# tmuird/VAEUNET

Hardware: AMD Instinct MI355X
Metric: images/sec (whole node) at 3x512x512 bs=8/GPU; Dice parity vs CPU ref (higher is better)
Workload: dtype bf16; 1 GPU; UNet(3,2) train step (fwd+CombinedLoss+bwd+clip+AdamW), random-init weights; image=3x512x512, batch_per_gpu=8, global_batch=8, parallelism=dp1, execution=hipgraph-replay, wgrad_side_stream=False

## Files before the change

vaeunet_amd/csrc/bn.hip:

```cpp
#include <cstdlib>
#include <type_traits>

#include "host.h"

namespace {

constexpr int STATS_TPB = 32;
constexpr int STATS_MAXS = 256;

__global__ void bn_stats_stage1(const float* psum, const float* pm2, int tiles, int64_t tile_rows,
                                int64_t rows, int C, int S, double* ws) {
  __shared__ double sh[4][64];
  const int cl = threadIdx.x & 63, tl = threadIdx.x >> 6;
  const int c = blockIdx.x * 64 + cl;
  const bool ok = c < C;
  const int per = (tiles + S - 1) / S;
  const int tb0 = blockIdx.y * per, te0 = min(tiles, tb0 + per);
  constexpr int U = STATS_TPB / 4;
  double N = 0, Mn = 0, Q = 0;
  for (int tb = tb0; tb < te0; tb += STATS_TPB) {
    const int te = min(te0, tb + STATS_TPB);
    const int64_t n_r = min(rows, (int64_t)te * tile_rows) - (int64_t)tb * tile_rows;
    float sv[U], mv[U];
    double nv[U];
    const int cc = ok ? c : 0;
#pragma unroll
    for (int u = 0; u < U; ++u) {
      const int t = min(tb + tl + 4 * u, te - 1);
      sv[u] = psum[(int64_t)t * C + cc];
      mv[u] = pm2[(int64_t)t * C + cc];
    }
#pragma unroll
    for (int u = 0; u < U; ++u) {
      const int t = tb + tl + 4 * u;
      const bool in = ok && t < te;
      sv[u] = in ? sv[u] : 0.f;
      mv[u] = in ? mv[u] : 0.f;
      int64_t nt = rows - (int64_t)t * tile_rows;
      nv[u] = in ? (double)(nt > tile_rows ? tile_rows : nt) : 0.0;
    }
    double s = 0;
#pragma unroll
    for (int u = 0; u < U; ++u) s += (double)sv[u];
    sh[tl][cl] = s;
    __syncthreads();
    const double m = (sh[0][cl] + sh[1][cl] + sh[2][cl] + sh[3][cl]) / (double)n_r;
    __syncthreads();
    double q = 0;
#pragma unroll
    for (int u = 0; u < U; ++u) {
      if (nv[u] > 0) {
        const double d = (double)sv[u] / nv[u] - m;
        q += (double)mv[u] + nv[u] * d * d;
      }
    }
    sh[tl][cl] = q;
// ... 41 lines not shown
  }
  double n = 0, sm = 0;
#pragma unroll
  for (int u = 0; u < U; ++u) { n += nv[u]; sm += nv[u] * mv[u]; }
  sh[0][q][cl] = n; sh[1][q][cl] = sm;
  __syncthreads();
#pragma unroll
  for (int w = 16; w >= 1; w >>= 1) {
    if (q < w) { sh[0][q][cl] += sh[0][q + w][cl]; sh[1][q][cl] += sh[1][q + w][cl]; }
    __syncthreads();
  }
  n = sh[0][0][cl];
  const double m = n > 0 ? sh[1][0][cl] / n : 0.0;
  __syncthreads();
  double M2 = 0;
#pragma unroll
  for (int u = 0; u < U; ++u) { const double d = mv[u] - m; M2 += qv[u] + nv[u] * d * d; }
  sh[0][q][cl] = M2;
  __syncthreads();
#pragma unroll
  for (int w = 16; w >= 1; w >>= 1) {
    if (q < w) sh[0][q][cl] += sh[0][q + w][cl];
    __syncthreads();
  }
  if (q != 0 || !ok) return;
  M2 = sh[0][0][cl];
  double var = n > 0 ? M2 / n : 0.0;
  float invstd = (float)(1.0 / sqrt(var + (double)eps));
  float mean = (float)m;
  scale[c] = g * invstd;
  shift[c] = b - mean * g * invstd;
  if (smean) smean[c] = mean;
  if (sinvstd) sinvstd[c] = invstd;
  if (nbt && c == 0) nbt[0] = nb0 + 1;
  if (upd) {
    double unb = n > 1 ? M2 / (n - 1) : var;
    rmean[c] = (1.f - momentum) * rm0 + momentum * mean;
    rvar[c] = (1.f - momentum) * rv0 + momentum * (float)unb;
  }
}

__global__ void bn_eval_kernel(const float* gamma, const float* beta, const float* rm, const float* rv,
                               float eps, int C, float* scale, float* shift, float* smean, float* sinvstd) {
  int c = blockIdx.x * blockDim.x + threadIdx.x;
  if (c >= C) return;
  float invstd = 1.f / sqrtf(rv[c] + eps);
  float g = gamma ? gamma[c] : 1.f, b = beta ? beta[c] : 0.f;
  scale[c] = g * invstd;
  shift[c] = b - rm[c] * g * invstd;
  if (smean) smean[c] = rm[c];
  if (sinvstd) sinvstd[c] = invstd;
}

struct ChanMap {
  int V, R, cv, row;
  VU_DEV ChanMap(int C) {
    V = C >> 3;
    R = 256 / V;
    cv = threadIdx.x & (V - 1);
    row = threadIdx.x / V;
  }
};

constexpr int UNR = 4;

template <typename T, bool NT>
__global__ void bn_apply_kernel(const T* x, int64_t xs, T* y, int64_t ys, int64_t P, int C,
                                const float* scale, const float* shift, int relu) {
  ChanMap cm(C);
  const int c = cm.cv * 8;
  float sc[8], sh[8];
#pragma unroll
  for (int i = 0; i < 8; ++i) { sc[i] = scale[c + i]; sh[i] = shift[c + i]; }
  const int64_t step = (int64_t)gridDim.x * cm.R * UNR;
  for (int64_t p0 = (int64_t)blockIdx.x * cm.R * UNR + cm.row; p0 < P; p0 += step) {
    Vec8<T> v[UNR];
#pragma unroll
    for (int u = 0; u < UNR; ++u) {
      const int64_t p = p0 + (int64_t)u * cm.R;
      if (p < P) { if (NT) v[u].load_nt(x + p * xs + c); else v[u].load(x + p * xs + c); }
    }
#pragma unroll
    for (int u = 0; u < UNR; ++u) {
      const int64_t p = p0 + (int64_t)u * cm.R;
      if (p >= P) continue;
#pragma unroll
      for (int i = 0; i < 8; ++i) {
        float z = v[u].get(i) * sc[i] + sh[i];
        v[u].set(i, relu ? fmaxf(z, 0.f) : z);
      }
      v[u].store(y + p * ys + c);
    }
  }
}

constexpr int RED_MAXBLK = 1024;

struct RedArgs {
  const void* a; int64_t as;
  const void* b; int64_t bs;
  int64_t P; int C;
  const float* scale; const float* shift; const float* mean; const float* invstd;
  int relu;
  float* part;
  int H, W, y0, x0, Hr, Wr;
};

VU_DEV int64_t win_pix(const RedArgs& r, int64_t p) {
  if (r.Hr == 0) return p;
  int64_t j = p % r.Wr, t = p / r.Wr;
  int64_t i = t % r.Hr, n = t / r.Hr;
  return (n * r.H + r.y0 + i) * r.W + r.x0 + j;
}

template <typename T, int MODE, bool NT>
__global__ void chan_partial_kernel(RedArgs r) {
  __shared__ float sh[2][256 * 8];
  ChanMap cm(r.C);
  const int c = cm.cv * 8;
  float s0[8], s1[8], sc[8], sf[8], mu[8], is[8];
#pragma unroll
  for (int i = 0; i < 8; ++i) {
    s0[i] = 0.f; s1[i] = 0.f;
    if (MODE == 1) {
      sc[i] = r.scale[c + i]; sf[i] = r.shift[c + i]; mu[i] = r.mean[c + i]; is[i] = r.invstd[c + i];
    }
  }
  const int64_t step = (int64_t)gridDim.x * cm.R * UNR;
  for (int64_t p0 = (int64_t)blockIdx.x * cm.R * UNR + cm.row; p0 < r.P; p0 += step) {
    Vec8<T> va[UNR], vb[UNR];
#pragma unroll
    for (int u = 0; u < UNR; ++u) {
      const int64_t p = p0 + (int64_t)u * cm.R;
      if (p < r.P) {
        const T* pa = reinterpret_cast<const T*>(r.a) + (MODE == 0 ? win_pix(r, p) : p) * r.as + c;
        const T* pb = reinterpret_cast<const T*>(r.b) + p * r.bs + c;
        if (NT) {
          va[u].load_nt(pa);
          if (MODE == 1) vb[u].load_nt(pb);
        } else {
          va[u].load(pa);
          if (MODE == 1) vb[u].load(pb);
        }
      }
    }
#pragma unroll
    for (int u = 0; u < UNR; ++u) {
      if (p0 + (int64_t)u * cm.R >= r.P) continue;
      if (MODE == 0) {
#pragma unroll
        for (int i = 0; i < 8; ++i) s0[i] += va[u].get(i);
      } else {
#pragma unroll
        for (int i = 0; i < 8; ++i) {
          float xv = vb[u].get(i);
          float dz = va[u].get(i);
          if (r.relu && !(fmaf(xv, sc[i], sf[i]) > 0.f)) dz = 0.f;
          s0[i] += dz;
          s1[i] += dz * ((xv - mu[i]) * is[i]);
        }
      }
    }
  }
#pragma unroll
  for (int i = 0; i < 8; ++i) { sh[0][cm.row * r.C + c + i] = s0[i]; sh[1][cm.row * r.C + c + i] = s1[i]; }
  __syncthreads();
  for (int cc = threadIdx.x; cc < r.C; cc += 256) {
    float a0 = 0.f, a1 = 0.f;
    a0 = lds_sum(&sh[0][cc], cm.R, r.C);
// ... 179 lines not shown
    st1<T>(dx + p * dxs + c, fmaf(coef[c], dz, coef[C + c] * (xv - mean[c])) + coef[2 * C + c]);
  }
}

template <typename T>
__global__ void bn_apply_scalar(const T* x, int64_t xs, T* y, int64_t ys, int64_t P, int C,
                                const float* scale, const float* shift, int relu) {
  int64_t tot = P * C;
  for (int64_t e = (int64_t)blockIdx.x * blockDim.x + threadIdx.x; e < tot;
       e += (int64_t)gridDim.x * blockDim.x) {
    int64_t p = e / C;
    int c = (int)(e - p * C);
    float z = ld1<T>(x + p * xs + c) * scale[c] + shift[c];
    st1<T>(y + p * ys + c, relu ? fmaxf(z, 0.f) : z);
  }
}

template <typename T>
__global__ void bn_apply_maxpool_kernel(const T* y, int64_t ys, T* a, int64_t as, T* pool, int64_t ps, int N,
                                        int H, int W, int C, const float* scale, const float* shift, int relu) {
  ChanMap cm(C);
  const int c = cm.cv * 8;
  float sc[8], sh[8];
#pragma unroll
  for (int i = 0; i < 8; ++i) { sc[i] = scale[c + i]; sh[i] = shift[c + i]; }
  const int Ho = H >> 1, Wo = W >> 1;
  const int64_t Q = (int64_t)N * Ho * Wo;
  for (int64_t q = (int64_t)blockIdx.x * cm.R + cm.row; q < Q; q += (int64_t)gridDim.x * cm.R) {
    const int j = (int)(q % Wo);
    const int64_t t = q / Wo;
    const int i = (int)(t % Ho), n = (int)(t / Ho);
    const int64_t p00 = ((int64_t)n * H + 2 * i) * W + 2 * j;
    Vec8<T> v[4];
#pragma unroll
    for (int k = 0; k < 4; ++k) v[k].load(y + (p00 + (k >> 1) * W + (k & 1)) * ys + c);
    float best[8];
#pragma unroll
    for (int e = 0; e < 8; ++e) best[e] = -INFINITY;
#pragma unroll
    for (int k = 0; k < 4; ++k) {
#pragma unroll
      for (int e = 0; e < 8; ++e) {
        const float z = v[k].get(e) * sc[e] + sh[e];
        v[k].set(e, relu ? fmaxf(z, 0.f) : z);
        const float f = v[k].get(e);
        if (f > best[e] || isnan(f)) best[e] = f;
      }
      v[k].store(a + (p00 + (k >> 1) * W + (k & 1)) * as + c);
    }
    Vec8<T> o;
#pragma unroll
    for (int e = 0; e < 8; ++e) o.set(e, best[e]);
    o.store(pool + q * ps + c);
  }
}

struct PoolBnArgs {
  const void* y; int64_t ys;
  const void* dp; int64_t dps;
  const void* add; int64_t adds;
  int N, H, W, C;
  const float* scale; const float* shift; const float* mean; const float* invstd;
  int relu;
  float* part;
  const float* coef;
  void* dx; int64_t dxs;
};

template <typename T, bool NT>
VU_DEV void pool_window(const PoolBnArgs& r, int64_t q, int c, const float (&sc)[8], const float (&sf)[8],
                        float (&yv)[4][8], float (&dz)[4][8], int64_t& p00) {
  const int Wo = r.W >> 1, Ho = r.H >> 1;
  const int j = (int)(q % Wo);
  const int64_t t = q / Wo;
  const int i = (int)(t % Ho), n = (int)(t / Ho);
  p00 = ((int64_t)n * r.H + 2 * i) * r.W + 2 * j;
  const T* y = reinterpret_cast<const T*>(r.y);
  const T* ad = reinterpret_cast<const T*>(r.add);
  Vec8<T> vy[4], va[4], vg;
#pragma unroll
  for (int k = 0; k < 4; ++k) {
    const int64_t pix = p00 + (k >> 1) * r.W + (k & 1);
    if (NT) vy[k].load_nt(y + pix * r.ys + c); else vy[k].load(y + pix * r.ys + c);
    if (ad) { if (NT) va[k].load_nt(ad + pix * r.adds + c); else va[k].load(ad + pix * r.adds + c); }
  }
  vg.load(reinterpret_cast<const T*>(r.dp) + q * r.dps + c);
  float best[8];
  int arg[8];
#pragma unroll
  for (int e = 0; e < 8; ++e) { best[e] = -INFINITY; arg[e] = 0; }
#pragma unroll
  for (int k = 0; k < 4; ++k)
#pragma unroll
    for (int e = 0; e < 8; ++e) {
      yv[k][e] = vy[k].get(e);
      const float z = fmaf(yv[k][e], sc[e], sf[e]);
      const float f = rnd<T>(r.relu ? fmaxf(z, 0.f) : z);
      if (f > best[e] || isnan(f)) { best[e] = f; arg[e] = k; }
    }
#pragma unroll
  for (int k = 0; k < 4; ++k)
#pragma unroll
    for (int e = 0; e < 8; ++e) {
      float o = ad ? va[k].get(e) : 0.f;
      if (arg[e] == k) o += vg.get(e);
      float d = rnd<T>(o);
      if (r.relu && !(fmaf(yv[k][e], sc[e], sf[e]) > 0.f)) d = 0.f;
      dz[k][e] = d;
    }
}

template <typename T, bool NT>
__global__ void pool_bn_partial_kernel(PoolBnArgs r) {
  __shared__ float sh[2][256 * 8];
  ChanMap cm(r.C);
  const int c = cm.cv * 8;
  float s0[8], s1[8], sc[8], sf[8], mu[8], is[8];
#pragma unroll
  for (int e = 0; e < 8; ++e) {
    s0[e] = 0.f; s1[e] = 0.f;
    sc[e] = r.scale[c + e]; sf[e] = r.shift[c + e]; mu[e] = r.mean[c + e]; is[e] = r.invstd[c + e];
  }
  const int64_t Q = (int64_t)r.N * (r.H >> 1) * (r.W >> 1);
  for (int64_t q = (int64_t)blockIdx.x * cm.R + cm.row; q < Q; q += (int64_t)gridDim.x * cm.R) {
    float yv[4][8], dz[4][8];
    int64_t p00;
    pool_window<T, NT>(r, q, c, sc, sf, yv, dz, p00);
#pragma unroll
    for (int k = 0; k < 4; ++k)
#pragma unroll
      for (int e = 0; e < 8; ++e) {
        s0[e] += dz[k][e];
        s1[e] += dz[k][e] * ((yv[k][e] - mu[e]) * is[e]);
      }
  }
#pragma unroll
  for (int e = 0; e < 8; ++e) { sh[0][cm.row * r.C + c + e] = s0[e]; sh[1][cm.row * r.C + c + e] = s1[e]; }
  __syncthreads();
  for (int cc = threadIdx.x; cc < r.C; cc += 256) {
    float a0 = 0.f, a1 = 0.f;
    a0 = lds_sum(&sh[0][cc], cm.R, r.C);
    a1 = lds_sum(&sh[1][cc], cm.R, r.C);
    r.part[((int64_t)blockIdx.x * 2 + 0) * r.C + cc] = a0;
    r.part[((int64_t)blockIdx.x * 2 + 1) * r.C + cc] = a1;
  }
}

template <typename T, bool NT>
__global__ void pool_bn_apply_kernel(PoolBnArgs r) {
  ChanMap cm(r.C);
  const int c = cm.cv * 8;
  float sc[8], sf[8], mu[8], k1[8], k2[8], k3[8];
#pragma unroll
  for (int e = 0; e < 8; ++e) {
    sc[e] = r.scale[c + e]; sf[e] = r.shift[c + e]; mu[e] = r.mean[c + e];
    k1[e] = r.coef[c + e]; k2[e] = r.coef[r.C + c + e]; k3[e] = r.coef[2 * r.C + c + e];
  }
  T* dx = reinterpret_cast<T*>(r.dx);
  const int64_t Q = (int64_t)r.N * (r.H >> 1) * (r.W >> 1);
  for (int64_t q = (int64_t)blockIdx.x * cm.R + cm.row; q < Q; q += (int64_t)gridDim.x * cm.R) {
    float yv[4][8], dz[4][8];
    int64_t p00;
    pool_window<T, NT>(r, q, c, sc, sf, yv, dz, p00);
#pragma unroll
    for (int k = 0; k < 4; ++k) {
      Vec8<T> vo;
#pragma unroll
      for (int e = 0; e < 8; ++e) vo.set(e, k1[e] * dz[k][e] + k2[e] * (yv[k][e] - mu[e]) + k3[e]);
      vo.store(dx + (p00 + (k >> 1) * r.W + (k & 1)) * r.dxs + c);
    }
  }
}

constexpr int BNF_MAXT = 256;

struct BnFusedArgs {
  const float* psum; const float* pm2; int tiles; int64_t tile_rows; int64_t P; int C;
  const float* gamma; const float* beta; float* rmean; float* rvar; int64_t* nbt; float momentum; float eps;
  float* coef;
  const void* y; int64_t ys;
  const void* res; int64_t rs; const float* rsc; const float* rsh;
  void* out; int64_t os; int relu; int split;
};

template <typename T>
__global__ __launch_bounds__(256) void bn_fwd_fused_kernel(BnFusedArgs a) {
  __shared__ double shd[8][32];
  __shared__ float ssc[32], ssh[32];
  const int cg = blockIdx.x / a.split, sp = blockIdx.x - cg * a.split;
  const int tid = threadIdx.x;
  {
    const int cl = tid & 31, tl = tid >> 5;
    const int c = cg * 32 + cl;
    const float g = a.gamma ? a.gamma[c] : 1.f, b = a.beta ? a.beta[c] : 0.f;
    const bool upd = sp == 0 && a.rmean && a.momentum != 0.f;
    const float rm0 = upd ? a.rmean[c] : 0.f, rv0 = upd ? a.rvar[c] : 0.f;
    const int64_t nb0 = (sp == 0 && a.nbt) ? a.nbt[0] : 0;
    constexpr int U = BNF_MAXT / 8;
    float sv[U], mv[U];
#pragma unroll
    for (int u = 0; u < U; ++u) {
      const int t = min(tl + 8 * u, a.tiles - 1);
      sv[u] = a.psum[(int64_t)t * a.C + c];
      mv[u] = a.pm2[(int64_t)t * a.C + c];
    }
    double s = 0.0;
#pragma unroll
    for (int u = 0; u < U; ++u) s += tl + 8 * u < a.tiles ? (double)sv[u] : 0.0;
    shd[tl][cl] = s;
    __syncthreads();
    double tot = 0.0;
#pragma unroll
    for (int k = 0; k < 8; ++k) tot += shd[k][cl];
    const double m = tot / (double)a.P;
    __syncthreads();
    double q = 0.0;
#pragma unroll
    for (int u = 0; u < U; ++u) {
      const int t = tl + 8 * u;
      if (t < a.tiles) {
        const int64_t nt64 = a.P - (int64_t)t * a.tile_rows;
        const double nt = (double)(nt64 > a.tile_rows ? a.tile_rows : nt64);
        const double d = (double)sv[u] / nt - m;
// ... 34 lines not shown
#pragma unroll
  for (int i = 0; i < 8; ++i) {
    sc[i] = ssc[cv * 8 + i];
    sh[i] = ssh[cv * 8 + i];
    rsc[i] = 1.f;
    rsh[i] = 0.f;
  }
  if (a.rsc) {
#pragma unroll
    for (int i = 0; i < 8; ++i) {
      rsc[i] = a.rsc[c + i];
      rsh[i] = a.rsh[c + i];
    }
  }
  const int64_t per = (a.P + a.split - 1) / a.split;
  const int64_t p_beg = (int64_t)sp * per, p_end = min(a.P, p_beg + per);
  const T* y = reinterpret_cast<const T*>(a.y);
  const T* r = reinterpret_cast<const T*>(a.res);
  T* out = reinterpret_cast<T*>(a.out);
  for (int64_t p0 = p_beg + row; p0 < p_end; p0 += 64 * UNR) {
    Vec8<T> vy[UNR], vr[UNR];
#pragma unroll
    for (int u = 0; u < UNR; ++u) {
      const int64_t p = p0 + (int64_t)u * 64 < p_end ? p0 + (int64_t)u * 64 : p_end - 1;
      vy[u].load(y + p * a.ys + c);
    }
    if (r) {
#pragma unroll
      for (int u = 0; u < UNR; ++u) {
        const int64_t p = p0 + (int64_t)u * 64 < p_end ? p0 + (int64_t)u * 64 : p_end - 1;
        vr[u].load(r + p * a.rs + c);
      }
    }
#pragma unroll
    for (int u = 0; u < UNR; ++u) {
      const int64_t p = p0 + (int64_t)u * 64;
      if (p >= p_end) continue;
      Vec8<T> vo;
#pragma unroll
      for (int i = 0; i < 8; ++i) {
        float z = vy[u].get(i) * sc[i] + sh[i];
        if (r) {
          float rr = vr[u].get(i);
          if (a.rsc) rr = rr * rsc[i] + rsh[i];
          z = z + rr;
        }
        vo.set(i, a.relu ? fmaxf(z, 0.f) : z);
      }
      vo.store(out + p * a.os + c);
    }
  }
}

constexpr int BNB_FUSED_MAXBLK = 128;

struct BnBwdFusedArgs {
  const void* dy; int64_t dys; const void* x; int64_t xs; int64_t P; int C;
  const float* scale; const float* shift; const float* mean; const float* invstd; const float* gamma;
  int relu; int train; const float* part; int nblk;
  float* dgamma; float* dbeta; int accumulate;
  void* dx; int64_t dxs; int split;
};

template <typename T>
__global__ __launch_bounds__(256) void bn_bwd_fused_apply_kernel(BnBwdFusedArgs a) {
  __shared__ double shd[2][8][32];
  __shared__ float sk[3][32];
  const int cg = blockIdx.x / a.split, sp = blockIdx.x - cg * a.split;
  const int tid = threadIdx.x;
  {
    const int cl = tid & 31, tl = tid >> 5;
    const int c = cg * 32 + cl;
    const float g = a.gamma ? a.gamma[c] : 1.f;
    const float is = a.invstd[c];
    const bool wr = sp == 0 && a.accumulate;
    const float dg0 = (wr && a.dgamma) ? a.dgamma[c] : 0.f;
    const float db0 = (wr && a.dbeta) ? a.dbeta[c] : 0.f;
    double s0 = 0.0, s1 = 0.0;
    for (int r0 = tl; r0 < a.nblk; r0 += 64) {
      float v0[8], v1[8];
#pragma unroll
      for (int u = 0; u < 8; ++u) {
        const int r = min(r0 + 8 * u, a.nblk - 1);
        v0[u] = a.part[((int64_t)r * 2 + 0) * a.C + c];
        v1[u] = a.part[((int64_t)r * 2 + 1) * a.C + c];
      }
#pragma unroll
      for (int u = 0; u < 8; ++u)
        if (r0 + 8 * u < a.nblk) {
          s0 += (double)v0[u];
          s1 += (double)v1[u];
        }
    }
    shd[0][tl][cl] = s0;
    shd[1][tl][cl] = s1;
    __syncthreads();
    if (tl == 0) {
      double S0 = 0.0, S1 = 0.0;
#pragma unroll
      for (int k = 0; k < 8; ++k) {
        S0 += shd[0][k][cl];
        S1 += shd[1][k][cl];
      }
      const float k1 = g * is;
      sk[0][cl] = k1;
      sk[1][cl] = a.train ? (float)(-(double)k1 * is * S1 / (double)a.P) : 0.f;
      sk[2][cl] = a.train ? (float)(-(double)k1 * S0 / (double)a.P) : 0.f;
      if (sp == 0) {
        if (a.dgamma) a.dgamma[c] = a.accumulate ? dg0 + (float)S1 : (float)S1;
        if (a.dbeta) a.dbeta[c] = a.accumulate ? db0 + (float)S0 : (float)S0;
      }
    }
    __syncthreads();
  }
  const int cv = tid & 3, row = tid >> 2;
  const int c = cg * 32 + cv * 8;
  float sc[8], sf[8], mu[8], k1[8], k2[8], k3[8];
#pragma unroll
  for (int i = 0; i < 8; ++i) {
    sc[i] = a.scale[c + i];
    sf[i] = a.shift[c + i];
    mu[i] = a.mean[c + i];
    k1[i] = sk[0][cv * 8 + i];
    k2[i] = sk[1][cv * 8 + i];
    k3[i] = sk[2][cv * 8 + i];
  }
  const int64_t per = (a.P + a.split - 1) / a.split;
  const int64_t p_beg = (int64_t)sp * per, p_end = min(a.P, p_beg + per);
  const T* dy = reinterpret_cast<const T*>(a.dy);
  const T* x = reinterpret_cast<const T*>(a.x);
  T* dx = reinterpret_cast<T*>(a.dx);
  for (int64_t p0 = p_beg + row; p0 < p_end; p0 += 64 * UNR) {
    Vec8<T> vd[UNR], vx[UNR];
#pragma unroll
    for (int u = 0; u < UNR; ++u) {
      const int64_t p = p0 + (int64_t)u * 64;
      if (p < p_end) {
        vd[u].load(dy + p * a.dys + c);
        vx[u].load(x + p * a.xs + c);
      }
    }
#pragma unroll
    for (int u = 0; u < UNR; ++u) {
      const int64_t p = p0 + (int64_t)u * 64;
      if (p >= p_end) continue;
      Vec8<T> vo;
#pragma unroll
      for (int i = 0; i < 8; ++i) {
        const float xv = vx[u].get(i);
        float dz = vd[u].get(i);
        if (a.relu && !(fmaf(xv, sc[i], sf[i]) > 0.f)) dz = 0.f;
        vo.set(i, fmaf(k1[i], dz, k2[i] * (xv - mu[i])) + k3[i]);
      }
      vo.store(dx + p * a.dxs + c);
    }
  }
}

inline bool chanmap_ok(int C, int64_t s0, int64_t s1, int64_t s2 = 0) {
  return C % 8 == 0 && pow2(C / 8) && C / 8 <= 256 && s0 % 8 == 0 && s1 % 8 == 0 && s2 % 8 == 0;
}

inline unsigned chan_grid16(int64_t P, int C, int maxblk) {
  int R = 256 / (C / 8);
  int64_t g = (P + (int64_t)R * 16 - 1) / ((int64_t)R * 16);
  if (g > maxblk) g = maxblk;
  if (g < 1) g = 1;
  return (unsigned)g;
}

inline unsigned chan_grid(int64_t P, int C, int maxblk) {
  int R = 256 / (C / 8);
  int64_t g = (P + (int64_t)R * 16 - 1) / ((int64_t)R * 16);
  const int64_t g1 = (P + (int64_t)R * UNR - 1) / ((int64_t)R * UNR);
  const int64_t minblk = tune(VU_TUNE_BN_MINBLK);
  const int64_t lo = g1 < minblk ? g1 : minblk;
  if (g < lo) g = lo;
  if (g > maxblk) g = maxblk;
  if (g < 1) g = 1;
  return (unsigned)g;
}

inline bool bn_nt(int64_t P, int C, int esize) {
  const int64_t mb = tune(VU_TUNE_BN_NT_MB);
  return mb >= 0 && P * C * esize >= mb * 1000000;
}

typedef void (*ApplyFn)(const bf16_t*, int64_t, bf16_t*, int64_t, int64_t, int, const float*, const float*, int);
typedef void (*BwdApplyFn)(const bf16_t*, int64_t, const bf16_t*, int64_t, int64_t, int, const float*,
                           const float*, const float*, const float*, int, bf16_t*, int64_t);
inline ApplyFn bn_apply_bf16(int64_t P, int C) {
  return bn_nt(P, C, 2) ? bn_apply_kernel<bf16_t, true> : bn_apply_kernel<bf16_t, false>;
}
inline BwdApplyFn bn_bwd_apply_bf16(int64_t P, int C) {
  return bn_nt(P, C, 2) ? bn_bwd_apply_kernel<bf16_t, true> : bn_bwd_apply_kernel<bf16_t, false>;
}

template <typename T, int MODE>
int launch_partial(const RedArgs& r, hipStream_t st, int& nblk, int maxblk = RED_MAXBLK) {
  bool vec = chanmap_ok(r.C, r.as, MODE == 0 ? 8 : r.bs);
  if (vec) {
    nblk = (int)chan_grid(r.P, r.C, maxblk);
    if (std::is_same<T, bf16_t>::value && bn_nt(r.P, r.C, 2))
      hipLaunchKernelGGL((chan_partial_kernel<T, MODE, true>), dim3(nblk), dim3(256), 0, st, r);
    else
      hipLaunchKernelGGL((chan_partial_kernel<T, MODE, false>), dim3(nblk), dim3(256), 0, st, r);
  } else if (r.C <= 256) {
    int R = 256 / r.C;
    int64_t g = (r.P + (int64_t)R * 16 - 1) / ((int64_t)R * 16);
    nblk = (int)(g > RED_MAXBLK ? RED_MAXBLK : (g < 1 ? 1 : g));
    hipLaunchKernelGGL((chan_partial_scalar<T, MODE>), dim3(nblk), dim3(256), 0, st, r);
  } else {
    return (int)hipErrorInvalidValue;
  }
  return (int)hipGetLastError();
}

}

extern "C" int64_t vu_reduce_workspace_bytes(int64_t P, int C) {
  (void)P;
  return (int64_t)RED_MAXBLK * 2 * C * (int64_t)sizeof(float);
}

static int stats_blocks(int tiles) {
  int S = (tiles + STATS_TPB - 1) / STATS_TPB;
  if (S > STATS_MAXS) S = STATS_MAXS;
  if (S < 1) S = 1;
  return S;
}

extern "C" int64_t vu_bn_finalize_workspace_bytes(int tiles, int C) {
  int S = stats_blocks(tiles);
  return (int64_t)S * C * 3 * sizeof(double);
}

extern "C" int vu_bn_finalize(const float* psum, const float* pm2, int tiles, int64_t tile_rows,
                              int64_t rows, int C, const float* gamma, const float* beta,
// ... 152 lines not shown
  const unsigned grid = chan_grid(P, C, 8192);
  if (dtype == VU_BF16) {
    if (bn_nt(P, C, 2))
      hipLaunchKernelGGL((bn_bwd_apply2_kernel<bf16_t, true>), dim3(grid), dim3(256), 0, st, (const bf16_t*)dy, dys,
                         (const bf16_t*)x1, x1s, (const bf16_t*)x2, x2s, P, C, mean1, coef1, mean2, coef2,
                         (bf16_t*)dx1, dx1s, (bf16_t*)dx2, dx2s);
    else
      hipLaunchKernelGGL((bn_bwd_apply2_kernel<bf16_t, false>), dim3(grid), dim3(256), 0, st, (const bf16_t*)dy,
                         dys, (const bf16_t*)x1, x1s, (const bf16_t*)x2, x2s, P, C, mean1, coef1, mean2, coef2,
                         (bf16_t*)dx1, dx1s, (bf16_t*)dx2, dx2s);
  } else {
    hipLaunchKernelGGL((bn_bwd_apply2_kernel<float, false>), dim3(grid), dim3(256), 0, st, (const float*)dy, dys,
                       (const float*)x1, x1s, (const float*)x2, x2s, P, C, mean1, coef1, mean2, coef2, (float*)dx1,
                       dx1s, (float*)dx2, dx2s);
  }
  return (int)hipGetLastError();
}

extern "C" int vu_chan_sum(const void* x, int64_t stride, int N, int H, int W, int y0, int x0, int Hr,
                           int Wr, int C, float* out, int accumulate, float* workspace, int dtype,
                           void* stream) {
  hipStream_t st = (hipStream_t)stream;
  int64_t P = (int64_t)N * Hr * Wr;
  RedArgs r{x, stride, nullptr, 0, P, C, nullptr, nullptr, nullptr, nullptr, 0, workspace, H, W, y0, x0, Hr, Wr};
  int nblk = 0, rc;
  rc = dtype == VU_BF16 ? launch_partial<bf16_t, 0>(r, st, nblk) : launch_partial<float, 0>(r, st, nblk);
  if (rc) return rc;
  hipLaunchKernelGGL(chan_final_sum, dim3((C + 31) / 32), dim3(COLSUM_THREADS), 0, st, workspace, nblk, C, out,
                     accumulate);
  return (int)hipGetLastError();
}

static bool pool_fusable(int H, int W, int C, int64_t s0, int64_t s1, int64_t s2) {
  return H % 2 == 0 && W % 2 == 0 && chanmap_ok(C, s0, s1, s2);
}

extern "C" int vu_bn_apply_maxpool2(const void* y, int64_t ys, void* a, int64_t as, void* pool, int64_t ps, int N,
                                    int H, int W, int C, const float* scale, const float* shift, int relu, int dtype,
                                    void* stream) {
  if (!pool_fusable(H, W, C, ys, as, ps)) return (int)hipErrorInvalidValue;
  const int64_t Q = (int64_t)N * (H / 2) * (W / 2);
  if (Q == 0) return 0;
  const unsigned grid = chan_grid(Q * 4, C, 8192);
  hipStream_t st = (hipStream_t)stream;
  if (dtype == VU_BF16)
    hipLaunchKernelGGL(bn_apply_maxpool_kernel<bf16_t>, dim3(grid), dim3(256), 0, st, (const bf16_t*)y, ys,
                       (bf16_t*)a, as, (bf16_t*)pool, ps, N, H, W, C, scale, shift, relu);
  else
    hipLaunchKernelGGL(bn_apply_maxpool_kernel<float>, dim3(grid), dim3(256), 0, st, (const float*)y, ys,
                       (float*)a, as, (float*)pool, ps, N, H, W, C, scale, shift, relu);
  return (int)hipGetLastError();
}

extern "C" int vu_bn_bwd_pool_supported(int H, int W, int C, int64_t ys, int64_t dps, int64_t adds, int64_t dxs) {
  return H % 2 == 0 && W % 2 == 0 && H > 0 && W > 0 && chanmap_ok(C, ys, dps, adds) && dxs % 8 == 0;
}

extern "C" int vu_bn_bwd_pool(const void* y, int64_t ys, const void* dp, int64_t dps, const void* add, int64_t adds,
                              int N, int H, int W, int C, const float* scale, const float* shift, const float* mean,
                              const float* invstd, const float* gamma, int relu, int train, float* dgamma,
                              float* dbeta, int accumulate, float* coef, float* workspace, void* dx, int64_t dxs,
                              int dtype, void* stream) {
  if (!vu_bn_bwd_pool_supported(H, W, C, ys, dps, add ? adds : 8, dxs) || N < 1) return (int)hipErrorInvalidValue;
  hipStream_t st = (hipStream_t)stream;
  const int64_t P = (int64_t)N * H * W;
  PoolBnArgs r{y, ys, dp, dps, add, adds, N, H, W, C, scale, shift, mean, invstd, relu, workspace, coef, dx, dxs};
  const int nblk = (int)chan_grid(P, C, RED_MAXBLK);
  const bool nt = bn_nt(P, C, dtype == VU_BF16 ? 2 : 4);
  const unsigned agrid = chan_grid(P, C, 8192);
  if (dtype == VU_BF16) {
    if (nt) hipLaunchKernelGGL((pool_bn_partial_kernel<bf16_t, true>), dim3(nblk), dim3(256), 0, st, r);
    else hipLaunchKernelGGL((pool_bn_partial_kernel<bf16_t, false>), dim3(nblk), dim3(256), 0, st, r);
  } else {
    hipLaunchKernelGGL((pool_bn_partial_kernel<float, false>), dim3(nblk), dim3(256), 0, st, r);
  }
  hipLaunchKernelGGL(bn_bwd_final, dim3((C + 31) / 32), dim3(COLSUM_THREADS), 0, st, workspace, nblk, C, P, gamma,
                     invstd, dgamma, dbeta, accumulate, coef, train);
  if (dtype == VU_BF16) {
    if (nt) hipLaunchKernelGGL((pool_bn_apply_kernel<bf16_t, true>), dim3(agrid), dim3(256), 0, st, r);
    else hipLaunchKernelGGL((pool_bn_apply_kernel<bf16_t, false>), dim3(agrid), dim3(256), 0, st, r);
  } else {
    hipLaunchKernelGGL((pool_bn_apply_kernel<float, false>), dim3(agrid), dim3(256), 0, st, r);
  }
  return (int)hipGetLastError();
}

extern "C" int vu_bn_fwd_fused_supported(int tiles, int C, int64_t ys, int64_t rs, int64_t os) {
  return tiles >= 1 && tiles <= BNF_MAXT && C % 32 == 0 && ys % 8 == 0 && rs % 8 == 0 && os % 8 == 0;
}

extern "C" int vu_bn_fwd_fused(const float* psum, const float* pm2, int tiles, int64_t tile_rows, int64_t P, int C,
                               const float* gamma, const float* beta, float* running_mean, float* running_var,
                               int64_t* num_batches_tracked, float momentum, float eps, float* coef, const void* y,
                               int64_t ys, const void* res, int64_t rs, const float* rscale, const float* rshift,
                               void* out, int64_t os, int relu, int dtype, void* stream) {
  if (!vu_bn_fwd_fused_supported(tiles, C, ys, res ? rs : 0, os) || P < 1) return (int)hipErrorInvalidValue;
  if ((rscale == nullptr) != (rshift == nullptr)) return (int)hipErrorInvalidValue;
  BnFusedArgs a{psum, pm2, tiles, tile_rows, P, C, gamma, beta, running_mean, running_var, num_batches_tracked,
                momentum, eps, coef, y, ys, res, rs, rscale, rshift, out, os, relu, 1};
  const int groups = C / 32;
  int64_t split = (256 + groups - 1) / groups;
  const int64_t maxs = (P + 127) / 128;
  if (split > maxs) split = maxs;
  if (split < 1) split = 1;
  a.split = (int)split;
  hipStream_t st = (hipStream_t)stream;
  if (dtype == VU_BF16)
    hipLaunchKernelGGL(bn_fwd_fused_kernel<bf16_t>, dim3((unsigned)(groups * split)), dim3(256), 0, st, a);
  else
    hipLaunchKernelGGL(bn_fwd_fused_kernel<float>, dim3((unsigned)(groups * split)), dim3(256), 0, st, a);
  return (int)hipGetLastError();
}

constexpr int ONEPASS_T = 512, ONEPASS_B = 8, ONEPASS_MAXP = 8192;
constexpr int ONEPASS_W = ONEPASS_T / 64;

VU_DEV float bfly_sum64(float v) {
#pragma unroll
  for (int m = 1; m < 64; m <<= 1) v += __shfl_xor(v, m, 64);
  return v;
}

template <typename T>
__global__ __launch_bounds__(ONEPASS_T) void bn_bwd_onepass_kernel(BnBwdFusedArgs a) {
  __shared__ float wsum[2][ONEPASS_W][8];
  __shared__ float sk[3][8];
  const int tid = threadIdx.x, lane = tid & 63, wv = tid >> 6;
  const int c = blockIdx.x * 8;
  const int P = (int)a.P, dys = (int)a.dys, xs = (int)a.xs;
  const T* dyc = reinterpret_cast<const T*>(a.dy) + c;
  const T* xc = reinterpret_cast<const T*>(a.x) + c;
  float sc[8], sf[8], mu[8], is[8], s0[8], s1[8];
#pragma unroll
  for (int i = 0; i < 8; ++i) {
    sc[i] = a.scale[c + i]; sf[i] = a.shift[c + i]; mu[i] = a.mean[c + i]; is[i] = a.invstd[c + i];
    s0[i] = 0.f; s1[i] = 0.f;
  }
  const bool wr = a.accumulate && tid < 8;
  const float g = tid < 8 ? (a.gamma ? a.gamma[c + tid] : 1.f) : 0.f;
// ... 120 lines not shown
```

Measured before the change: 563.9 images/sec.

## Restructure pooled BN backward into per-pixel partial sweep and relu-specialized kernels

Moves the maxpool+BN backward kernels into their own file and reworks the partial-reduction kernel to iterate per full-resolution pixel with unrolled pairs instead of per pooling window. ReLU is now a template parameter, and launch bounds are added. For small problems the partial grid is capped at the fused max block count, and finalization goes through a shared finish helper. This aims to improve memory-level parallelism and cut divergence, at the cost of redundantly reloading the 2x2 window for each pixel in the partial pass.

```diff
diff --git a/vaeunet_amd/csrc/bn.hip b/vaeunet_amd/csrc/bn.hip
--- a/vaeunet_amd/csrc/bn.hip
+++ b/vaeunet_amd/csrc/bn.hip
@@ -2,6 +2,7 @@
 #include <type_traits>
 
 #include "host.h"
+#include "bn_stream.h"
 
 namespace {
 
@@ -149,18 +150,6 @@
   if (sinvstd) sinvstd[c] = invstd;
 }
 
-struct ChanMap {
-  int V, R, cv, row;
-  VU_DEV ChanMap(int C) {
-    V = C >> 3;
-    R = 256 / V;
-    cv = threadIdx.x & (V - 1);
-    row = threadIdx.x / V;
-  }
-};
-
-constexpr int UNR = 4;
-
 template <typename T, bool NT>
 __global__ void bn_apply_kernel(const T* x, int64_t xs, T* y, int64_t ys, int64_t P, int C,
                                 const float* scale, const float* shift, int relu) {
@@ -191,7 +180,6 @@
   }
 }
 
-constexpr int RED_MAXBLK = 1024;
 
 struct RedArgs {
   const void* a; int64_t as;
@@ -211,7 +199,7 @@
 }
 
 template <typename T, int MODE, bool NT>
-__global__ void chan_partial_kernel(RedArgs r) {
+__global__ __launch_bounds__(256) void chan_partial_kernel(RedArgs r) {
   __shared__ float sh[2][256 * 8];
   ChanMap cm(r.C);
   const int c = cm.cv * 8;
@@ -497,123 +485,6 @@
 #pragma unroll
     for (int e = 0; e < 8; ++e) o.set(e, best[e]);
     o.store(pool + q * ps + c);
-  }
-}
-
-struct PoolBnArgs {
-  const void* y; int64_t ys;
-  const void* dp; int64_t dps;
-  const void* add; int64_t adds;
-  int N, H, W, C;
-  const float* scale; const float* shift; const float* mean; const float* invstd;
-  int relu;
-  float* part;
-  const float* coef;
-  void* dx; int64_t dxs;
-};
-
-template <typename T, bool NT>
-VU_DEV void pool_window(const PoolBnArgs& r, int64_t q, int c, const float (&sc)[8], const float (&sf)[8],
-                        float (&yv)[4][8], float (&dz)[4][8], int64_t& p00) {
-  const int Wo = r.W >> 1, Ho = r.H >> 1;
-  const int j = (int)(q % Wo);
-  const int64_t t = q / Wo;
-  const int i = (int)(t % Ho), n = (int)(t / Ho);
-  p00 = ((int64_t)n * r.H + 2 * i) * r.W + 2 * j;
-  const T* y = reinterpret_cast<const T*>(r.y);
-  const T* ad = reinterpret_cast<const T*>(r.add);
-  Vec8<T> vy[4], va[4], vg;
-#pragma unroll
-  for (int k = 0; k < 4; ++k) {
-    const int64_t pix = p00 + (k >> 1) * r.W + (k & 1);
-    if (NT) vy[k].load_nt(y + pix * r.ys + c); else vy[k].load(y + pix * r.ys + c);
-    if (ad) { if (NT) va[k].load_nt(ad + pix * r.adds + c); else va[k].load(ad + pix * r.adds + c); }
-  }
-  vg.load(reinterpret_cast<const T*>(r.dp) + q * r.dps + c);
-  float best[8];
-  int arg[8];
-#pragma unroll
-  for (int e = 0; e < 8; ++e) { best[e] = -INFINITY; arg[e] = 0; }
-#pragma unroll
-  for (int k = 0; k < 4; ++k)
-#pragma unroll
-    for (int e = 0; e < 8; ++e) {
-      yv[k][e] = vy[k].get(e);
-      const float z = fmaf(yv[k][e], sc[e], sf[e]);
-      const float f = rnd<T>(r.relu ? fmaxf(z, 0.f) : z);
-      if (f > best[e] || isnan(f)) { best[e] = f; arg[e] = k; }
-    }
-#pragma unroll
-  for (int k = 0; k < 4; ++k)
-#pragma unroll
-    for (int e = 0; e < 8; ++e) {
-      float o = ad ? va[k].get(e) : 0.f;
-      if (arg[e] == k) o += vg.get(e);
-      float d = rnd<T>(o);
-      if (r.relu && !(fmaf(yv[k][e], sc[e], sf[e]) > 0.f)) d = 0.f;
-      dz[k][e] = d;
-    }
-}
-
-template <typename T, bool NT>
-__global__ void pool_bn_partial_kernel(PoolBnArgs r) {
-  __shared__ float sh[2][256 * 8];
-  ChanMap cm(r.C);
-  const int c = cm.cv * 8;
-  float s0[8], s1[8], sc[8], sf[8], mu[8], is[8];
-#pragma unroll
-  for (int e = 0; e < 8; ++e) {
-    s0[e] = 0.f; s1[e] = 0.f;
-    sc[e] = r.scale[c + e]; sf[e] = r.shift[c + e]; mu[e] = r.mean[c + e]; is[e] = r.invstd[c + e];
-  }
-  const int64_t Q = (int64_t)r.N * (r.H >> 1) * (r.W >> 1);
-  for (int64_t q = (int64_t)blockIdx.x * cm.R + cm.row; q < Q; q += (int64_t)gridDim.x * cm.R) {
-    float yv[4][8], dz[4][8];
-    int64_t p00;
-    pool_window<T, NT>(r, q, c, sc, sf, yv, dz, p00);
-#pragma unroll
-    for (int k = 0; k < 4; ++k)
-#pragma unroll
-      for (int e = 0; e < 8; ++e) {
-        s0[e] += dz[k][e];
-        s1[e] += dz[k][e] * ((yv[k][e] - mu[e]) * is[e]);
-      }
-  }
-#pragma unroll
-  for (int e = 0; e < 8; ++e) { sh[0][cm.row * r.C + c + e] = s0[e]; sh[1][cm.row * r.C + c + e] = s1[e]; }
-  __syncthreads();
-  for (int cc = threadIdx.x; cc < r.C; cc += 256) {
-    float a0 = 0.f, a1 = 0.f;
-    a0 = lds_sum(&sh[0][cc], cm.R, r.C);
-    a1 = lds_sum(&sh[1][cc], cm.R, r.C);
-    r.part[((int64_t)blockIdx.x * 2 + 0) * r.C + cc] = a0;
-    r.part[((int64_t)blockIdx.x * 2 + 1) * r.C + cc] = a1;
-  }
-}
-
-template <typename T, bool NT>
-__global__ void pool_bn_apply_kernel(PoolBnArgs r) {
-  ChanMap cm(r.C);
-  const int c = cm.cv * 8;
-  float sc[8], sf[8], mu[8], k1[8], k2[8], k3[8];
-#pragma unroll
-  for (int e = 0; e < 8; ++e) {
-    sc[e] = r.scale[c + e]; sf[e] = r.shift[c + e]; mu[e] = r.mean[c + e];
-    k1[e] = r.coef[c + e]; k2[e] = r.coef[r.C + c + e]; k3[e] = r.coef[2 * r.C + c + e];
-  }
-  T* dx = reinterpret_cast<T*>(r.dx);
-  const int64_t Q = (int64_t)r.N * (r.H >> 1) * (r.W >> 1);
-  for (int64_t q = (int64_t)blockIdx.x * cm.R + cm.row; q < Q; q += (int64_t)gridDim.x * cm.R) {
-    float yv[4][8], dz[4][8];
-    int64_t p00;
-    pool_window<T, NT>(r, q, c, sc, sf, yv, dz, p00);
-#pragma unroll
-    for (int k = 0; k < 4; ++k) {
-      Vec8<T> vo;
-#pragma unroll
-      for (int e = 0; e < 8; ++e) vo.set(e, k1[e] * dz[k][e] + k2[e] * (yv[k][e] - mu[e]) + k3[e]);
-      vo.store(dx + (p00 + (k >> 1) * r.W + (k & 1)) * r.dxs + c);
-    }
   }
 }
 
@@ -754,7 +625,6 @@
   }
 }
 
-constexpr int BNB_FUSED_MAXBLK = 128;
 
 struct BnBwdFusedArgs {
   const void* dy; int64_t dys; const void* x; int64_t xs; int64_t P; int C;
@@ -859,33 +729,12 @@
   }
 }
 
-inline bool chanmap_ok(int C, int64_t s0, int64_t s1, int64_t s2 = 0) {
-  return C % 8 == 0 && pow2(C / 8) && C / 8 <= 256 && s0 % 8 == 0 && s1 % 8 == 0 && s2 % 8 == 0;
-}
-
 inline unsigned chan_grid16(int64_t P, int C, int maxblk) {
   int R = 256 / (C / 8);
   int64_t g = (P + (int64_t)R * 16 - 1) / ((int64_t)R * 16);
   if (g > maxblk) g = maxblk;
   if (g < 1) g = 1;
   return (unsigned)g;
-}
-
-inline unsigned chan_grid(int64_t P, int C, int maxblk) {
-  int R = 256 / (C / 8);
-  int64_t g = (P + (int64_t)R * 16 - 1) / ((int64_t)R * 16);
-  const int64_t g1 = (P + (int64_t)R * UNR - 1) / ((int64_t)R * UNR);
-  const int64_t minblk = tune(VU_TUNE_BN_MINBLK);
-  const int64_t lo = g1 < minblk ? g1 : minblk;
-  if (g < lo) g = lo;
-  if (g > maxblk) g = maxblk;
-  if (g < 1) g = 1;
-  return (unsigned)g;
-}
-
-inline bool bn_nt(int64_t P, int C, int esize) {
-  const int64_t mb = tune(VU_TUNE_BN_NT_MB);
-  return mb >= 0 && P * C * esize >= mb * 1000000;
 }
 
 typedef void (*ApplyFn)(const bf16_t*, int64_t, bf16_t*, int64_t, int64_t, int, const float*, const float*, int);
@@ -1144,39 +993,6 @@
   return (int)hipGetLastError();
 }
 
-extern "C" int vu_bn_bwd_pool_supported(int H, int W, int C, int64_t ys, int64_t dps, int64_t adds, int64_t dxs) {
-  return H % 2 == 0 && W % 2 == 0 && H > 0 && W > 0 && chanmap_ok(C, ys, dps, adds) && dxs % 8 == 0;
-}
-
-extern "C" int vu_bn_bwd_pool(const void* y, int64_t ys, const void* dp, int64_t dps, const void* add, int64_t adds,
-                              int N, int H, int W, int C, const float* scale, const float* shift, const float* mean,
-                              const float* invstd, const float* gamma, int relu, int train, float* dgamma,
-                              float* dbeta, int accumulate, float* coef, float* workspace, void* dx, int64_t dxs,
-                              int dtype, void* stream) {
-  if (!vu_bn_bwd_pool_supported(H, W, C, ys, dps, add ? adds : 8, dxs) || N < 1) return (int)hipErrorInvalidValue;
-  hipStream_t st = (hipStream_t)stream;
-  const int64_t P = (int64_t)N * H * W;
-  PoolBnArgs r{y, ys, dp, dps, add, adds, N, H, W, C, scale, shift, mean, invstd, relu, workspace, coef, dx, dxs};
-  const int nblk = (int)chan_grid(P, C, RED_MAXBLK);
-  const bool nt = bn_nt(P, C, dtype == VU_BF16 ? 2 : 4);
-  const unsigned agrid = chan_grid(P, C, 8192);
-  if (dtype == VU_BF16) {
-    if (nt) hipLaunchKernelGGL((pool_bn_partial_kernel<bf16_t, true>), dim3(nblk), dim3(256), 0, st, r);
-    else hipLaunchKernelGGL((pool_bn_partial_kernel<bf16_t, false>), dim3(nblk), dim3(256), 0, st, r);
-  } else {
-    hipLaunchKernelGGL((pool_bn_partial_kernel<float, false>), dim3(nblk), dim3(256), 0, st, r);
-  }
-  hipLaunchKernelGGL(bn_bwd_final, dim3((C + 31) / 32), dim3(COLSUM_THREADS), 0, st, workspace, nblk, C, P, gamma,
-                     invstd, dgamma, dbeta, accumulate, coef, train);
-  if (dtype == VU_BF16) {
-    if (nt) hipLaunchKernelGGL((pool_bn_apply_kernel<bf16_t, true>), dim3(agrid), dim3(256), 0, st, r);
-    else hipLaunchKernelGGL((pool_bn_apply_kernel<bf16_t, false>), dim3(agrid), dim3(256), 0, st, r);
-  } else {
-    hipLaunchKernelGGL((pool_bn_apply_kernel<float, false>), dim3(agrid), dim3(256), 0, st, r);
-  }
-  return (int)hipGetLastError();
-}
-
 extern "C" int vu_bn_fwd_fused_supported(int tiles, int C, int64_t ys, int64_t rs, int64_t os) {
   return tiles >= 1 && tiles <= BNF_MAXT && C % 32 == 0 && ys % 8 == 0 && rs % 8 == 0 && os % 8 == 0;
 }
diff --git a/vaeunet_amd/csrc/bn_pool.hip b/vaeunet_amd/csrc/bn_pool.hip
--- /dev/null
+++ b/vaeunet_amd/csrc/bn_pool.hip
@@ -0,0 +1,238 @@
+#include "host.h"
+#include "bn_stream.h"
+
+namespace {
+
+struct PoolBnArgs {
+  const void* y; int64_t ys;
+  const void* dp; int64_t dps;
+  const void* add; int64_t adds;
+  int N, H, W, C;
+  const float* scale; const float* shift; const float* mean; const float* invstd;
+  int relu;
+  float* part;
+  const float* coef;
+  void* dx; int64_t dxs;
+};
+
+template <typename T>
+struct PoolRows {
+  Vec8<T> y[4], a[4], g;
+  int64_t p00;
+};
+
+template <typename T, bool NT>
+VU_DEV void pool_load(const PoolBnArgs& r, int64_t q, int c, PoolRows<T>& w) {
+  const int Wo = r.W >> 1, Ho = r.H >> 1;
+  const int j = (int)(q % Wo);
+  const int64_t t = q / Wo;
+  const int i = (int)(t % Ho), n = (int)(t / Ho);
+  w.p00 = ((int64_t)n * r.H + 2 * i) * r.W + 2 * j;
+  const T* y = reinterpret_cast<const T*>(r.y);
+  const T* ad = reinterpret_cast<const T*>(r.add);
+#pragma unroll
+  for (int k = 0; k < 4; ++k) {
+    const int64_t pix = w.p00 + (k >> 1) * r.W + (k & 1);
+    if (NT) w.y[k].load_nt(y + pix * r.ys + c); else w.y[k].load(y + pix * r.ys + c);
+  }
+  if (ad) {
+#pragma unroll
+    for (int k = 0; k < 4; ++k) {
+      const int64_t pix = w.p00 + (k >> 1) * r.W + (k & 1);
+      if (NT) w.a[k].load_nt(ad + pix * r.adds + c); else w.a[k].load(ad + pix * r.adds + c);
+    }
+  } else {
+#pragma unroll
+    for (int k = 0; k < 4; ++k) w.a[k].zero();
+  }
+  w.g.load(reinterpret_cast<const T*>(r.dp) + q * r.dps + c);
+}
+
+template <typename T, bool RELU>
+VU_DEV void pool_dz(const PoolRows<T>& w, int e, float sc, float sf, float (&yv)[4], float (&dz)[4]) {
+  float best = -INFINITY;
+  int arg = 0;
+  bool pos[4];
+#pragma unroll
+  for (int k = 0; k < 4; ++k) {
+    yv[k] = w.y[k].get(e);
+    const float z = fmaf(yv[k], sc, sf);
+    pos[k] = z > 0.f;
+    const float f = rnd<T>(RELU ? fmaxf(z, 0.f) : z);
+    if (f > best || isnan(f)) { best = f; arg = k; }
+  }
+  const float g = w.g.get(e);
+#pragma unroll
+  for (int k = 0; k < 4; ++k) {
+    float o = w.a[k].get(e);
+    if (arg == k) o += g;
+    const float d = rnd<T>(o);
+    dz[k] = (RELU && !pos[k]) ? 0.f : d;
+  }
+}
+
+template <typename T>
+struct PoolPix {
+  Vec8<T> y[4], ys, a, g;
+  int self;
+};
+
+template <typename T, bool NT>
+VU_DEV void pool_pix_load(const PoolBnArgs& r, int64_t p, int c, PoolPix<T>& w) {
+  const int xx = (int)(p % r.W);
+  const int64_t t = p / r.W;
+  const int yy = (int)(t % r.H);
+  const int64_t n = t / r.H;
+  w.self = (yy & 1) * 2 + (xx & 1);
+  const int64_t p00 = p - (int64_t)(yy & 1) * r.W - (xx & 1);
+  const int64_t q = (n * (r.H >> 1) + (yy >> 1)) * (r.W >> 1) + (xx >> 1);
+  const T* y = reinterpret_cast<const T*>(r.y);
+  const T* ad = reinterpret_cast<const T*>(r.add);
+#pragma unroll
+  for (int k = 0; k < 4; ++k) {
+    const int64_t pix = p00 + (k >> 1) * r.W + (k & 1);
+    if (NT) w.y[k].load_nt(y + pix * r.ys + c); else w.y[k].load(y + pix * r.ys + c);
+  }
+  if (NT) w.ys.load_nt(y + p * r.ys + c); else w.ys.load(y + p * r.ys + c);
+  if (!ad) w.a.zero();
+  else if (NT) w.a.load_nt(ad + p * r.adds + c);
+  else w.a.load(ad + p * r.adds + c);
+  w.g.load(reinterpret_cast<const T*>(r.dp) + q * r.dps + c);
+}
+
+template <typename T, bool NT, bool RELU>
+VU_DEV void pool_partial_sweep(const PoolBnArgs& r, const ChanMap& cm, float (&s0)[8], float (&s1)[8]) {
+  const int c = cm.cv * 8;
+  float sc[8], sf[8], mu[8], is[8];
+#pragma unroll
+  for (int e = 0; e < 8; ++e) {
+    sc[e] = r.scale[c + e]; sf[e] = r.shift[c + e]; mu[e] = r.mean[c + e]; is[e] = r.invstd[c + e];
+  }
+  const int64_t P = (int64_t)r.N * r.H * r.W;
+  const int64_t step = (int64_t)gridDim.x * cm.R * UNR;
+  for (int64_t p0 = (int64_t)blockIdx.x * cm.R * UNR + cm.row; p0 < P; p0 += step) {
+#pragma unroll
+    for (int h = 0; h < UNR; h += 2) {
+      PoolPix<T> w[2];
+#pragma unroll
+      for (int u = 0; u < 2; ++u) {
+        const int64_t p = p0 + (int64_t)(h + u) * cm.R;
+        if (p < P) pool_pix_load<T, NT>(r, p, c, w[u]);
+      }
+#pragma unroll
+      for (int u = 0; u < 2; ++u) {
+        if (p0 + (int64_t)(h + u) * cm.R >= P) continue;
+#pragma unroll
+        for (int e = 0; e < 8; ++e) {
+          float best = -INFINITY;
+          int arg = 0;
+#pragma unroll
+          for (int k = 0; k < 4; ++k) {
+            const float z = fmaf(w[u].y[k].get(e), sc[e], sf[e]);
+            const float f = rnd<T>(RELU ? fmaxf(z, 0.f) : z);
+            if (f > best || isnan(f)) { best = f; arg = k; }
+          }
+          const float xv = w[u].ys.get(e);
+          float o = w[u].a.get(e);
+          if (arg == w[u].self) o += w[u].g.get(e);
+          float dz = rnd<T>(o);
+          if (RELU && !(fmaf(xv, sc[e], sf[e]) > 0.f)) dz = 0.f;
+          s0[e] += dz;
+          s1[e] += dz * ((xv - mu[e]) * is[e]);
+        }
+      }
+    }
+  }
+}
+
+template <typename T, bool NT>
+__global__ __launch_bounds__(256) void pool_bn_partial_kernel(PoolBnArgs r) {
+  __shared__ float sh[2][256 * 8];
+  ChanMap cm(r.C);
+  const int c = cm.cv * 8;
+  float s0[8], s1[8];
+#pragma unroll
+  for (int e = 0; e < 8; ++e) { s0[e] = 0.f; s1[e] = 0.f; }
+  if (r.relu) pool_partial_sweep<T, NT, true>(r, cm, s0, s1);
+  else pool_partial_sweep<T, NT, false>(r, cm, s0, s1);
+#pragma unroll
+  for (int e = 0; e < 8; ++e) { sh[0][cm.row * r.C + c + e] = s0[e]; sh[1][cm.row * r.C + c + e] = s1[e]; }
+  __syncthreads();
+  for (int cc = threadIdx.x; cc < r.C; cc += 256) {
+    float a0 = 0.f, a1 = 0.f;
+    a0 = lds_sum(&sh[0][cc], cm.R, r.C);
+    a1 = lds_sum(&sh[1][cc], cm.R, r.C);
+    r.part[((int64_t)blockIdx.x * 2 + 0) * r.C + cc] = a0;
+    r.part[((int64_t)blockIdx.x * 2 + 1) * r.C + cc] = a1;
+  }
+}
+
+template <typename T, bool NT, bool RELU>
+VU_DEV void pool_apply_sweep(const PoolBnArgs& r, const ChanMap& cm) {
+  const int c = cm.cv * 8;
+  float sc[8], sf[8], mu[8], k1[8], k2[8], k3[8];
+#pragma unroll
+  for (int e = 0; e < 8; ++e) {
+    sc[e] = r.scale[c + e]; sf[e] = r.shift[c + e]; mu[e] = r.mean[c + e];
+    k1[e] = r.coef[c + e]; k2[e] = r.coef[r.C + c + e]; k3[e] = r.coef[2 * r.C + c + e];
+  }
+  T* dx = reinterpret_cast<T*>(r.dx);
+  const int64_t Q = (int64_t)r.N * (r.H >> 1) * (r.W >> 1);
+  for (int64_t q = (int64_t)blockIdx.x * cm.R + cm.row; q < Q; q += (int64_t)gridDim.x * cm.R) {
+    PoolRows<T> w;
+    pool_load<T, NT>(r, q, c, w);
+#pragma unroll
+    for (int e = 0; e < 8; ++e) {
+      float yv[4], dz[4];
+      pool_dz<T, RELU>(w, e, sc[e], sf[e], yv, dz);
+#pragma unroll
+      for (int k = 0; k < 4; ++k) w.a[k].set(e, fmaf(k1[e], dz[k], k2[e] * (yv[k] - mu[e])) + k3[e]);
+    }
+#pragma unroll
+    for (int k = 0; k < 4; ++k) w.a[k].store(dx + (w.p00 + (k >> 1) * r.W + (k & 1)) * r.dxs + c);
+  }
+}
+
+template <typename T, bool NT>
+__global__ __launch_bounds__(256) void pool_bn_apply_kernel(PoolBnArgs r) {
+  ChanMap cm(r.C);
+  if (r.relu) pool_apply_sweep<T, NT, true>(r, cm);
+  else pool_apply_sweep<T, NT, false>(r, cm);
+}
+
+}
+
+extern "C" int vu_bn_bwd_pool_supported(int H, int W, int C, int64_t ys, int64_t dps, int64_t adds, int64_t dxs) {
+  return H % 2 == 0 && W % 2 == 0 && H > 0 && W > 0 && chanmap_ok(C, ys, dps, adds) && dxs % 8 == 0;
+}
+
+extern "C" int vu_bn_bwd_pool(const void* y, int64_t ys, const void* dp, int64_t dps, const void* add, int64_t adds,
+                              int N, int H, int W, int C, const float* scale, const float* shift, const float* mean,
+                              const float* invstd, const float* gamma, int relu, int train, float* dgamma,
+                              float* dbeta, int accumulate, float* coef, float* workspace, void* dx, int64_t dxs,
+                              int dtype, void* stream) {
+  if (!vu_bn_bwd_pool_supported(H, W, C, ys, dps, add ? adds : 8, dxs) || N < 1) return (int)hipErrorInvalidValue;
+  hipStream_t st = (hipStream_t)stream;
+  const int64_t P = (int64_t)N * H * W;
+  PoolBnArgs r{y, ys, dp, dps, add, adds, N, H, W, C, scale, shift, mean, invstd, relu, workspace, coef, dx, dxs};
+  const bool small = vu_bn_bwd_fused_supported(P, C, 8, ys, dxs) != 0;
+  const int nblk = (int)chan_grid(P, C, small ? BNB_FUSED_MAXBLK : RED_MAXBLK);
+  const bool nt = bn_nt(P, C, dtype == VU_BF16 ? 2 : 4);
+  const unsigned agrid = chan_grid(P, C, 8192);
+  if (dtype == VU_BF16) {
+    if (nt) hipLaunchKernelGGL((pool_bn_partial_kernel<bf16_t, true>), dim3(nblk), dim3(256), 0, st, r);
+    else hipLaunchKernelGGL((pool_bn_partial_kernel<bf16_t, false>), dim3(nblk), dim3(256), 0, st, r);
+  } else {
+    hipLaunchKernelGGL((pool_bn_partial_kernel<float, false>), dim3(nblk), dim3(256), 0, st, r);
+  }
+  int rc = vu_bn_bwd_finish(workspace, nblk, P, C, gamma, invstd, train, dgamma, dbeta, accumulate, coef, nullptr,
+                            stream);
+  if (rc) return rc;
+  if (dtype == VU_BF16) {
+    if (nt) hipLaunchKernelGGL((pool_bn_apply_kernel<bf16_t, true>), dim3(agrid), dim3(256), 0, st, r);
+    else hipLaunchKernelGGL((pool_bn_apply_kernel<bf16_t, false>), dim3(agrid), dim3(256), 0, st, r);
+  } else {
+    hipLaunchKernelGGL((pool_bn_apply_kernel<float, false>), dim3(agrid), dim3(256), 0, st, r);
+  }
+  return (int)hipGetLastError();
+}
diff --git a/vaeunet_amd/csrc/bn_stream.h b/vaeunet_amd/csrc/bn_stream.h
--- /dev/null
+++ b/vaeunet_amd/csrc/bn_stream.h
@@ -0,0 +1,38 @@
+#pragma once
+#include "host.h"
+
+struct ChanMap {
+  int V, R, cv, row;
+  VU_DEV ChanMap(int C) {
+    V = C >> 3;
+    R = 256 / V;
+    cv = threadIdx.x & (V - 1);
+    row = threadIdx.x / V;
+  }
+};
+
+constexpr int UNR = 4;
+
+constexpr int RED_MAXBLK = 1024;
+constexpr int BNB_FUSED_MAXBLK = 128;
+
+inline bool chanmap_ok(int C, int64_t s0, int64_t s1, int64_t s2 = 0) {
+  return C % 8 == 0 && pow2(C / 8) && C / 8 <= 256 && s0 % 8 == 0 && s1 % 8 == 0 && s2 % 8 == 0;
+}
+
+inline unsigned chan_grid(int64_t P, int C, int maxblk) {
+  int R = 256 / (C / 8);
+  int64_t g = (P + (int64_t)R * 16 - 1) / ((int64_t)R * 16);
+  const int64_t g1 = (P + (int64_t)R * UNR - 1) / ((int64_t)R * UNR);
+  const int64_t minblk = tune(VU_TUNE_BN_MINBLK);
+  const int64_t lo = g1 < minblk ? g1 : minblk;
+  if (g < lo) g = lo;
+  if (g > maxblk) g = maxblk;
+  if (g < 1) g = 1;
+  return (unsigned)g;
+}
+
+inline bool bn_nt(int64_t P, int C, int esize) {
+  const int64_t mb = tune(VU_TUNE_BN_NT_MB);
+  return mb >= 0 && P * C * esize >= mb * 1000000;
+}
```

Measured after the change: 564.0 images/sec (median of 5 runs). No clear change (+0.0%).
